# JoshuaLim007/VoxelEngine

Hardware: AMD Instinct MI355X
Metric: Mrays/s primary+1-bounce @1080p, 8k×512×8k brickmap; % HBM roofline (higher is better)
Workload: dtype f32

## Files before the change

### include/vxrt.h

```cpp
#ifndef VXRT_H
#define VXRT_H

#include <stddef.h>
#include <stdint.h>

#ifdef __cplusplus
extern "C" {
#endif

#define VXRT_ABI_VERSION 3
#define VXRT_EMPTY_SLOT 0xFFFFFFFFu
#define VXRT_MAX_STEPS 2048

typedef enum vxrt_status {
    VXRT_OK = 0,
    VXRT_ERR_INVALID = -1,
    VXRT_ERR_HIP = -2,
    VXRT_ERR_NO_WORLD = -3,
    VXRT_ERR_NOMEM = -4
} vxrt_status;

typedef struct vxrt_ctx vxrt_ctx;

int vxrt_abi_version(void);
int vxrt_create(int device, vxrt_ctx **out);
int vxrt_destroy(vxrt_ctx *ctx);
const char *vxrt_last_error(void);
int vxrt_synchronize(vxrt_ctx *ctx);
int vxrt_set_kernel_variant(vxrt_ctx *ctx, int variant);
int vxrt_debug_guard_pretend_no_slack(vxrt_ctx *ctx, int on);
int vxrt_has_experiments(void);
int vxrt_set_persistent_waves_per_cu(vxrt_ctx *ctx, int waves_per_cu);

typedef struct vxrt_world_desc {
    uint32_t struct_size;
    int32_t factor;
    int32_t cdims[3];
    uint64_t nslots;
    const uint32_t *coarse_bits;
    const uint32_t *brick_slot;
    const float *bounds;
    const uint32_t *pool;
} vxrt_world_desc;
int vxrt_upload_world(vxrt_ctx *ctx, const vxrt_world_desc *desc);

// ... 219 lines not shown
```

### voxelengine_amd/_native.py

```python
from __future__ import annotations

import ctypes as C
import os

from . import build as _build

EMPTY_SLOT = 0xFFFFFFFF
MAX_STEPS = 2048
GEN_HASH_HEIGHTFIELD, GEN_PERLIN_REF, GEN_INT_TERRAIN = 0, 1, 2
MODE_SHADED, MODE_DEBUG = 0, 1

EXPORTS = [
    "vxrt_abi_version", "vxrt_create", "vxrt_destroy", "vxrt_last_error", "vxrt_synchronize", "vxrt_set_kernel_variant", "vxrt_kernel_for_launch",
    "vxrt_has_experiments", "vxrt_set_persistent_waves_per_cu", "vxrt_debug_guard_pretend_no_slack",
    "vxrt_upload_world", "vxrt_build_world_procedural", "vxrt_world_info_get", "vxrt_download_world",
    "vxrt_save_world", "vxrt_load_world", "vxrt_world_file_info",
    "vxrt_set_environment", "vxrt_set_fov", "vxrt_set_ortho_window_size", "vxrt_get_directions",
    "vxrt_render_flags_default", "vxrt_render", "vxrt_render_views", "vxrt_compact_rows", "vxrt_frame_stats_get",
    "vxrt_deinterleave_strips", "vxrt_deinterleave_views", "vxrt_trace_batch", "vxrt_trace_batch_host",
    "vxrt_set_batch_max_steps", "vxrt_stream_open", "vxrt_stream_focus", "vxrt_stream_resident", "vxrt_stream_close",
    "vxrt_edit_voxels", "vxrt_edit_reserve",
    "vxrt_region_words", "vxrt_read_region", "vxrt_read_region_host", "vxrt_edit_stamps",
    "vxrt_move_boxes", "vxrt_overlap_boxes", "vxrt_move_boxes_host", "vxrt_overlap_boxes_host",
    "vxrt_islands_workspace_bytes", "vxrt_find_islands", "vxrt_find_islands_host",
    "vxrt_nav_workspace_bytes", "vxrt_nav_field", "vxrt_nav_paths", "vxrt_nav_field_host",
    "vxrt_distance_workspace_bytes", "vxrt_distance_field", "vxrt_distance_field_host",
]
EDIT_BOX, EDIT_SPHERE = 0, 1
EDIT_MAX_OPS = 1024
# ... 94 lines not shown
    path = os.environ.get("VXRT_LIB", _build.LIB_PATH)
    if path == _build.LIB_PATH:
        _build.build_lib(force=bool(os.environ.get("VXRT_REBUILD")))
    if not os.path.exists(path):
        raise RuntimeError(f"libvxrt.so not found at {path}; run __graft_entry__.build()")
    L = C.CDLL(path)
    f3 = C.POINTER(C.c_float)
    L.vxrt_abi_version.restype = C.c_int
    L.vxrt_last_error.restype = C.c_char_p
    L.vxrt_create.argtypes = [C.c_int, C.POINTER(C.c_void_p)]
    L.vxrt_destroy.argtypes = [C.c_void_p]
    L.vxrt_synchronize.argtypes = [C.c_void_p]
    L.vxrt_set_kernel_variant.argtypes = [C.c_void_p, C.c_int]
    L.vxrt_has_experiments.restype = C.c_int
    L.vxrt_debug_guard_pretend_no_slack.argtypes = [C.c_void_p, C.c_int]
    L.vxrt_set_persistent_waves_per_cu.argtypes = [C.c_void_p, C.c_int]
    L.vxrt_kernel_for_launch.argtypes = [C.c_void_p, C.c_uint32, C.c_uint32, C.c_void_p, C.c_uint32]
    L.vxrt_kernel_for_launch.restype = C.c_int
    L.vxrt_upload_world.argtypes = [C.c_void_p, C.POINTER(WorldDesc)]
    L.vxrt_build_world_procedural.argtypes = [C.c_void_p, C.c_int, C.c_int, C.c_int, C.c_int, C.c_int]
    L.vxrt_world_info_get.argtypes = [C.c_void_p, C.POINTER(WorldInfo)]
    L.vxrt_download_world.argtypes = [C.c_void_p, C.c_void_p, C.c_void_p, C.c_void_p, C.c_void_p]
    L.vxrt_save_world.argtypes = [C.c_void_p, C.c_char_p]
    L.vxrt_load_world.argtypes = [C.c_void_p, C.c_char_p]
    L.vxrt_world_file_info.argtypes = [C.c_char_p, C.POINTER(WorldInfo)]
    L.vxrt_set_environment.argtypes = [C.c_void_p, f3, f3, f3]
    L.vxrt_set_fov.argtypes = [C.c_void_p, C.c_float]
    L.vxrt_set_ortho_window_size.argtypes = [C.c_void_p, C.c_float, C.c_float]
    L.vxrt_get_directions.argtypes = [f3, f3, f3, f3]
    L.vxrt_get_directions.restype = None
# ... 66 lines not shown
```

### voxelengine_amd/csrc/vxrt_api.hip

```cpp
#include "../../include/vxrt.h"
#include "vxrt_dist.hpp"
#include "vxrt_edit.hpp"
#include "vxrt_kernels.hpp"
#include "vxrt_islands.hpp"
#include "vxrt_nav.hpp"
#include "vxrt_region.hpp"
#include "vxrt_stream.hpp"

#include <algorithm>
#include <atomic>
#include <cmath>
#include <cstdio>
#include <cstdlib>
#include <cstring>
#include <initializer_list>
#include <map>
#include <new>
#include <set>
#include <string>
#include <utility>
#include <vector>

namespace vxrt {
hipError_t launch_render(const RenderArgs& A, bool stats, int variant, hipStream_t stream);
int resolve_render_variant(const RenderArgs& A, int variant);
hipError_t launch_trace_batch(const BatchArgs& B, bool stats, int variant, hipStream_t stream);
void launch_deinterleave(const void* shards, unsigned long long shard_stride_bytes, void* fb, uint32_t width,
                         uint32_t height, uint32_t strip_rows, uint32_t strip_count, hipStream_t stream, uint32_t n_views = 1,
                         unsigned long long view_stride_bytes = 0, unsigned long long fb_stride_bytes = 0);
int build_world_on_device(struct ::vxrt_ctx* ctx, int generator, int X, int Y, int Z, int factor);
hipError_t layout_bits(const uint32_t* src, uint32_t* dst, const int cd[3], bool to_hbm);
hipError_t layout_meta(const uint2* src, uint2* dst, const int cd[3], bool to_hbm);
hipError_t layout_bricks(const uint32_t* src, uint32_t* dst, uint64_t nbricks, int f, bool to_hbm);
hipError_t chunk_tables(uint2* meta, uint32_t* coarse, const uint2* d_chunk_meta, int tx, int ty, int tz, int cx, int cz);
hipError_t edit_bricks(const uint32_t* cells, uint32_t n, const EditOpDev* ops, uint32_t nops, const uint2* meta,
                       const uint32_t* pool, uint32_t* scratch, uint32_t* ext, uint2* info, int f, int cx, int cz);
hipError_t edit_commit(const uint32_t* cells, const uint32_t* new_slot, uint32_t n, const uint32_t* zero, uint32_t nzero,
                       const uint32_t* scratch, const uint32_t* ext, uint32_t* pool, uint2* meta, uint32_t* coarse, int f);
hipError_t gather_bricks(const uint32_t* pool, const uint32_t* idx, uint32_t n, uint32_t* dst, int f);
hipError_t stamp_bricks(const uint32_t* cells, uint32_t n, const StampDev* stamps, uint32_t nst, const uint2* meta,
                        const uint32_t* pool, uint32_t* scratch, uint32_t* ext, uint2* info, int f, int cx, int cz);
hipError_t move_boxes(const CollideWorld& W, const float* bodies, uint64_t n, const int order[3], float* lohi, uint32_t* flags,
                      hipStream_t stream);
hipError_t overlap_boxes(const CollideWorld& W, const float* bodies, uint64_t n, uint32_t* counts, uint32_t* flags,
                         hipStream_t stream);
hipError_t find_islands(const CollideWorld& W, const int32_t o[3], const int32_t d[3], uint32_t anchors, void* work,
                        uint32_t* floating, uint32_t* labels, vxrt_island* table, uint32_t max_islands,
                        vxrt_island_summary* summary, hipStream_t stream);
hipError_t nav_field(const CollideWorld& W, const int32_t o[3], const int32_t d[3], const vxrt_nav_agent& ag, const int32_t* goals,
// ... 15 lines not shown
#define VX_HIP(call)                                                                                   \
    do {                                                                                               \
        hipError_t e_ = (call);                                                                        \
        if (e_ != hipSuccess)                                                                          \
            return fail(VXRT_ERR_HIP, std::string(#call) + ": " + hipGetErrorString(e_));              \
    } while (0)

struct vxrt_ctx {
    int device = 0;
    bool has_world = false;
    vxrt::WorldView view{};
    uint32_t* d_coarse = nullptr;
    void* coarse_alloc = nullptr;
    void* pool_alloc = nullptr;
    uint2* d_meta = nullptr;
    uint32_t* d_pool = nullptr;
    uint64_t ncells = 0, nslots = 0, pool_capacity_slots = 0;
    uint64_t coarse_alloc_bytes = 0, pool_alloc_bytes = 0;
    bool guard_no_slack = false;
    float light_dir[3] = {0, 0, 0};
    float light_color[3] = {0, 0, 0};
    float ambient[3] = {0, 0, 0};
    float fov = 90.0f;
    float ortho[2] = {10.0f, 10.0f};
    uint32_t frame_counter = 0;
    int kernel_variant = 4;
    unsigned persistent_waves = 4096;
    unsigned cus = 256;
    unsigned long long* d_stats = nullptr;
    unsigned int* d_queues = nullptr;
// ... 27 lines not shown
};
constexpr unsigned kViewSlots = 16;
constexpr unsigned kTileCounterRing = 64;
static_assert(kTileCounterRing == sizeof(vxrt_ctx::counter_busy) / sizeof(hipEvent_t), "ring size");
static_assert(kViewSlots == sizeof(vxrt_ctx::views_busy) / sizeof(hipEvent_t), "ring size");

namespace vxrt {

void stream_drop(vxrt_ctx* c);

static void free_world(vxrt_ctx* c)
{
    stream_drop(c);
    if (c->coarse_alloc) (void)hipFree(c->coarse_alloc);
    if (c->d_meta) (void)hipFree(c->d_meta);
    if (c->pool_alloc) (void)hipFree(c->pool_alloc);
    c->coarse_alloc = c->pool_alloc = nullptr;
    c->d_coarse = nullptr;
    c->d_meta = nullptr;
    c->d_pool = nullptr;
    c->has_world = false;
    c->ncells = c->nslots = c->pool_capacity_slots = 0;
    c->free_slots.clear();
    c->edited = false;
}

int check_shape(int factor, const int cd[3])
{
    if (!(factor == 8 || factor == 16 || factor == 32))
        return fail(VXRT_ERR_INVALID, "factor must be 8, 16 or 32");
    for (int a = 0; a < 3; ++a)
        if (cd[a] <= 0 || cd[a] % 8 != 0 || cd[a] > 65535)
            return fail(VXRT_ERR_INVALID, "coarse dimensions must be positive multiples of 8 (the tables' tiled order)");
    const uint64_t slice = (uint64_t)cd[0] * (uint64_t)cd[2];
    if ((uint64_t)cd[1] * (uint64_t)cd[2] >= (1ull << 24) || slice * (uint64_t)cd[1] + 2ull * slice + 64ull >= (1ull << 32))
        return fail(VXRT_ERR_INVALID, "coarse grid too large for 32-bit cell indices (cy * cz must stay below 2^24, cx * cz * (cy + 2) below 2^32)");
    return VXRT_OK;
}

void fill_view(vxrt_ctx* c, int factor, const int cd[3])
{
    WorldView& v = c->view;
    v.coarse_bits = c->d_coarse;
    v.cell_meta = c->d_meta;
    v.pool = c->d_pool;
    v.cx = cd[0];
    v.cy = cd[1];
    v.cz = cd[2];
    v.c_row = cd[0];
    v.c_slice = cd[0] * cd[2];
    v.f = factor;
    v.f_row = factor;
    v.f_slice = factor * factor;
    v.brick_words = (uint32_t)(factor * factor * factor / 32);
    v.ff = (float)factor;
    v.inv_f = 1.0f / (float)factor;
    v.wmax_x = (float)((double)cd[0] - 1e-6);
    v.wmax_y = (float)((double)cd[1] - 1e-6);
    v.wmax_z = (float)((double)cd[2] - 1e-6);
// ... 11 lines not shown
static hipError_t alloc_pool(uint64_t bw, uint64_t slots, void** alloc, uint64_t* alloc_bytes, uint32_t** pool)
{
    const uint64_t pool_bytes = (slots ? slots : 1) * bw * sizeof(uint32_t);
    const uint64_t pool_slack = (bw * sizeof(uint32_t) + 255) / 256 * 256;
    hipError_t e = hipMalloc(alloc, pool_bytes + 2 * pool_slack);
    if (e != hipSuccess)
        return e;
    *alloc_bytes = pool_bytes + 2 * pool_slack;
    *pool = reinterpret_cast<uint32_t*>(static_cast<unsigned char*>(*alloc) + pool_slack);
    return hipSuccess;
}

int alloc_world(vxrt_ctx* c, int factor, const int cd[3], uint64_t pool_slots)
{
    free_world(c);
    c->ncells = (uint64_t)cd[0] * cd[1] * cd[2];
    uint64_t bw = (uint64_t)factor * factor * factor / 32;
    const uint64_t coarse_bytes = ((c->ncells + 31) / 32) * sizeof(uint32_t);
    const uint64_t coarse_slack = (((uint64_t)cd[0] * cd[2] / 8 + 64) + 255) / 256 * 256;
    VX_HIP(hipMalloc(&c->coarse_alloc, coarse_bytes + 2 * coarse_slack));
    c->coarse_alloc_bytes = coarse_bytes + 2 * coarse_slack;
    c->d_coarse = reinterpret_cast<uint32_t*>(static_cast<unsigned char*>(c->coarse_alloc) + coarse_slack);
    VX_HIP(hipMalloc((void**)&c->d_meta, c->ncells * sizeof(uint2)));
    VX_HIP(alloc_pool(bw, pool_slots, &c->pool_alloc, &c->pool_alloc_bytes, &c->d_pool));
    c->pool_capacity_slots = pool_slots;
    return VXRT_OK;
}

int adopt_world(vxrt_ctx* c, int factor, const int cd[3], uint64_t nslots, uint32_t** d_coarse, uint2** d_meta,
                uint32_t** d_pool)
{
    int rc = alloc_world(c, factor, cd, nslots);
    if (rc)
        return rc;
    c->nslots = nslots;
    fill_view(c, factor, cd);
    c->has_world = true;
    *d_coarse = c->d_coarse;
// ... 171 lines not shown
#endif
}

int vxrt_debug_guard_pretend_no_slack(vxrt_ctx* c, int on)
{
    if (!c)
        return fail(VXRT_ERR_INVALID, "NULL context");
    c->guard_no_slack = on != 0;
    if (c->has_world) {
        const int cd[3] = {c->view.cx, c->view.cy, c->view.cz};
        vxrt::fill_view(c, c->view.f, cd);
    }
    return VXRT_OK;
}

int vxrt_set_kernel_variant(vxrt_ctx* c, int variant)
{
    if (!c || !(variant == 1 || variant == 4 || variant == 7))
        return fail(VXRT_ERR_INVALID, "variant must be 4 (default), 7 (the persistent kernels on the wave-level tracer: what the default runs) or 1 (straightforward per-lane loops, the cross-check)");
    c->kernel_variant = variant;
    return VXRT_OK;
}

int vxrt_synchronize(vxrt_ctx* c)
{
    if (!c)
        return fail(VXRT_ERR_INVALID, "ctx is NULL");
    VX_HIP(hipSetDevice(c->device));
    VX_HIP(hipDeviceSynchronize());
    return VXRT_OK;
// ... 76 lines not shown
    return vxrt::build_world_on_device(c, generator, X, Y, Z, factor);
}

int vxrt_world_info_get(vxrt_ctx* c, vxrt_world_info* out)
{
    if (!c || !out)
        return fail(VXRT_ERR_INVALID, "NULL argument");
    if (!c->has_world)
        return fail(VXRT_ERR_NO_WORLD, "no world resident");
    out->factor = c->view.f;
    out->cdims[0] = c->view.cx;
    out->cdims[1] = c->view.cy;
    out->cdims[2] = c->view.cz;
    out->ncells = c->ncells;
    out->nslots = c->nslots;
    out->hbm_bytes = ((c->ncells + 31) / 32) * 4 + c->ncells * sizeof(uint2) + c->nslots * c->view.brick_words * 4ull;
    return VXRT_OK;
}

int vxrt_download_world(vxrt_ctx* c, uint32_t* coarse_bits, uint32_t* brick_slot, float* bounds, uint32_t* pool)
{
    if (!c || !coarse_bits || !brick_slot || !bounds)
        return fail(VXRT_ERR_INVALID, "NULL argument");
    if (!c->has_world)
        return fail(VXRT_ERR_NO_WORLD, "no world resident");
    VX_HIP(hipSetDevice(c->device));
    VX_HIP(hipDeviceSynchronize());
    const int cd[3] = {c->view.cx, c->view.cy, c->view.cz};
    const uint64_t coarse_bytes = ((c->ncells + 31) / 32) * sizeof(uint32_t);
    const uint64_t bw = c->view.brick_words;
    const uint64_t piece = std::max<uint64_t>(1, (64ull << 20) / (bw * 4));
// ... 136 lines not shown
    const unsigned n = nviews ? nviews : 1u;
    for (unsigned v = 0; v < n; ++v) {
        if (!views[v].d_fb)
            return fail(VXRT_ERR_INVALID, "a view has no framebuffer");
        for (int a = 0; a < 3; ++a)
            if (!std::isfinite(views[v].origin[a]) || !std::isfinite(views[v].fwd[a]) || !std::isfinite(views[v].up[a]) ||
                !std::isfinite(views[v].right[a]))
                return fail(VXRT_ERR_INVALID, "camera origin / forward / up / right must be finite numbers");
    }
    if (fl->d_accum && nviews != 0)
        return fail(VXRT_ERR_INVALID, "temporal accumulation (d_accum) is per view: use vxrt_render");
    if (fl->d_accum && (reinterpret_cast<uintptr_t>(fl->d_accum) & 15u))
        return fail(VXRT_ERR_INVALID, "d_accum must be 16-byte aligned");
    VX_HIP(hipSetDevice(c->device));
    hipStream_t stream = (hipStream_t)fl->stream;

    vxrt::RenderArgs A;
    memset(&A, 0, sizeof(A));
    A.W = c->view;
    A.width = width;
    A.height = height;
    {
        float aspect = (float)width / (float)height;
        float fov = (float)((double)c->fov * 3.1415 / 180.0);
        A.kx = tanf(fov / 2.0f) * aspect;
        A.ky = tanf(fov / 2.0f);
        A.ratio = (float)width / (float)height;
        A.ortho_x = c->ortho[0];
        A.ortho_y = c->ortho[1];
    }
// ... 206 lines not shown
                              (hipStream_t)stream, n_views, view_stride_bytes, fb_stride_bytes);
    VX_HIP(hipGetLastError());
    return VXRT_OK;
}

int vxrt_trace_batch(vxrt_ctx* c, const float* d_origins, const float* d_dirs, uint64_t n, float* d_pos,
                     float* d_normal, int32_t* d_steps, uint8_t* d_hit, int64_t* d_voxel, vxrt_frame_stats* stats,
                     void* stream_)
{
    if (!c || (n && (!d_origins || !d_dirs || !d_pos || !d_normal || !d_steps)))
        return fail(VXRT_ERR_INVALID, "NULL argument");
    if (!c->has_world)
        return fail(VXRT_ERR_NO_WORLD, "no world resident");
    VX_HIP(hipSetDevice(c->device));
    hipStream_t stream = (hipStream_t)stream_;
    vxrt::BatchArgs B;
    memset(&B, 0, sizeof(B));
    B.W = c->view;
    B.origins = d_origins;
    B.dirs = d_dirs;
    B.n = n;
    B.pos = d_pos;
    B.normal = d_normal;
    B.steps = d_steps;
    B.hit = d_hit;
    B.voxel = (long long*)d_voxel;
    B.stats = c->d_stats;
    const unsigned tslot = c->launch_seq.fetch_add(1u) % kTileCounterRing;
    bool capturing = false;
    VX_HIP(vxrt::ring_acquire(c->counter_busy[tslot], stream, capturing));
// ... 455 lines not shown
    vxrt::fill_view(c, h.factor, cd);
    c->has_world = true;
    c->stream = S;
    return VXRT_OK;
}

int vxrt_stream_focus(vxrt_ctx* c, const float focus[3], float radius, vxrt_stream_stats* out)
{
    if (!c || !focus || !vxrt::StreamPolicy::focus_valid(focus, radius))
        return fail(VXRT_ERR_INVALID, "NULL argument, non-finite focus, or negative or NaN radius");
    StreamState* S = c->stream;
    if (!S)
        return fail(VXRT_ERR_NO_WORLD, "no streamed world (vxrt_stream_open)");
    VX_HIP(hipSetDevice(c->device));
    VX_HIP(hipDeviceSynchronize());
    StreamDeviceIO io(c, S);
    vxrt::StreamPolicy::Result r;
    const int rc = S->P.focus(focus, radius, S->brick_bytes, io, r);
    const hipError_t e = hipDeviceSynchronize();
    if (rc)
        return rc;
    if (e != hipSuccess)
        return fail(VXRT_ERR_HIP, std::string("hipDeviceSynchronize: ") + hipGetErrorString(e));
    if (out) {
        out->chunks_total = S->P.nchunks;
        out->chunks_occupied = S->P.chunks_occupied;
        out->chunks_resident = S->P.chunks_resident;
        out->bricks_resident = S->P.bricks_resident;
        out->chunks_loaded = r.loaded;
        out->chunks_evicted = r.evicted;
// ... 44 lines not shown
        return fail(VXRT_ERR_NOMEM, std::string("brick pool growth to ") + std::to_string(capacity) + " bricks: " + hipGetErrorString(e));
    }
    if (c->nslots)
        e = hipMemcpy(pool, c->d_pool, c->nslots * bw * 4, hipMemcpyDeviceToDevice);
    if (e == hipSuccess)
        e = hipDeviceSynchronize();
    if (e != hipSuccess) {
        (void)hipFree(alloc);
        return fail(VXRT_ERR_HIP, std::string("brick pool growth: ") + hipGetErrorString(e));
    }
    (void)hipFree(c->pool_alloc);
    c->pool_alloc = alloc;
    c->pool_alloc_bytes = alloc_bytes;
    c->d_pool = pool;
    c->pool_capacity_slots = capacity;
    const int cd[3] = {c->view.cx, c->view.cy, c->view.cz};
    fill_view(c, c->view.f, cd);
    return VXRT_OK;
}

template <class Op>
static void edit_cells(const std::vector<Op>& ops, int f, int cx, int cz, uint64_t ncells, std::vector<uint32_t>& cells)
{
    uint64_t total = 0;
    for (const Op& op : ops) {
        uint64_t v = 1;
        for (int a = 0; a < 3; ++a)
            v *= (uint64_t)(op.hi[a] / f - op.lo[a] / f + 1);
        total += v;
    }
// ... 76 lines not shown
        flags[i] = (uint8_t)info[i].y;
    }
    EditPlan P;
    edit_plan_slots(old_slot.data(), flags.data(), n, c->free_slots, c->nslots, P);
    if (P.changed == 0)
        return finish();
    int rc = VXRT_OK;
    if (P.nslots >= (1ull << 32) - 2)
        rc = fail(VXRT_ERR_NOMEM, "brick slots exhausted (32-bit slot numbers)");
    else if (P.nslots > c->pool_capacity_slots)
        rc = grow_pool(c, edit_grown_capacity(c->pool_capacity_slots, P.nslots));
    if (rc) {
        edit_plan_undo(P, c->free_slots);
        return rc;
    }
    uint32_t* d_new = static_cast<uint32_t*>(c->edit_plan.p);
    uint32_t* d_zero = d_new + n;
    std::vector<uint32_t> plan(P.new_slot);
    plan.insert(plan.end(), P.zero.begin(), P.zero.end());
    e = hipMemcpy(d_new, plan.data(), plan.size() * 4, hipMemcpyHostToDevice);
    if (e == hipSuccess)
        e = edit_commit(d_cells, d_new, n, d_zero, (uint32_t)P.zero.size(), d_img, d_ext, c->d_pool, c->d_meta, c->d_coarse, f);
    if (e == hipSuccess)
        e = hipDeviceSynchronize();
    if (e != hipSuccess) {
        edit_plan_undo(P, c->free_slots);
        return fail(VXRT_ERR_HIP, std::string("edit commit: ") + hipGetErrorString(e));
    }
    c->nslots = P.nslots;
    c->edited = true;
// ... 506 lines not shown
```

### voxelengine_amd/csrc/vxrt_device.hpp

```cpp
#pragma once

#include <hip/hip_runtime.h>
#include <stdint.h>

namespace vxrt {

constexpr int kMaxSteps = 2048;
constexpr uint32_t kEmptySlot = 0xFFFFFFFFu;
constexpr float kInf = __builtin_huge_valf();
constexpr float kFltEps = 1.1920928955078125e-7f;

struct f3 {
    float x, y, z;
};
__device__ __forceinline__ f3 mk3(float x, float y, float z) { return f3{x, y, z}; }
__device__ __forceinline__ f3 operator+(f3 a, f3 b) { return f3{a.x + b.x, a.y + b.y, a.z + b.z}; }
__device__ __forceinline__ f3 operator-(f3 a, f3 b) { return f3{a.x - b.x, a.y - b.y, a.z - b.z}; }
__device__ __forceinline__ f3 operator*(f3 a, float s) { return f3{a.x * s, a.y * s, a.z * s}; }
__device__ __forceinline__ float dot3(f3 a, f3 b) { return a.x * b.x + a.y * b.y + a.z * b.z; }
__device__ __forceinline__ float lo(float a, float b) { return a < b ? a : b; }
__device__ __forceinline__ float hi(float a, float b) { return a > b ? a : b; }
__device__ __forceinline__ f3 unit3(f3 v) { return v * (1.0f / sqrtf(dot3(v, v))); }

#ifndef VXRT_HOST_CHECK
// ... 20 lines not shown
__device__ __forceinline__ float div_rn(float a, float b, float y)
{
    const float q = a * y;
    return fmaf(fmaf(-b, q, a), y, q);
}
__device__ __forceinline__ bool ordinary(float x)
{
    return ((__float_as_uint(x) & 0x7FFFFFFFu) - 0x0D800000u) < (0x72000000u - 0x0D800000u);
}
__device__ __forceinline__ f3 unit3_ordinary(f3 v, float dd) { return v * rcp_rn(sqrt_rn(dd)); }
__device__ __forceinline__ f3 reflect3(f3 i, f3 n) { return i - (n * 2.0f) * dot3(n, i); }

struct WorldView {
    const uint32_t* __restrict__ coarse_bits;
    const uint2* __restrict__ cell_meta;
    const uint32_t* __restrict__ pool;
    int cx, cy, cz;
    int c_row, c_slice;
    int f;
    int f_row, f_slice;
    uint32_t brick_words;
    float ff;
    float inv_f;
    float wmax_x, wmax_y, wmax_z;
    int X, Y;
    int c_wide;
    const uint32_t *coarse_end, *coarse_lo, *coarse_hi;
    const uint32_t *pool_end, *pool_lo, *pool_hi;
};

#ifndef VXRT_FIELD_CAP_XZ
#define VXRT_FIELD_CAP_XZ 1020u
#define VXRT_FIELD_CAP_Y 508u
#endif
constexpr uint32_t kFieldCapXZ = VXRT_FIELD_CAP_XZ, kFieldCapY = VXRT_FIELD_CAP_Y;

__host__ __device__ inline bool grid_is_wide(int cx, int cy, int cz)
{
    return cx > (int)kFieldCapXZ || cz > (int)kFieldCapXZ || cy > (int)kFieldCapY || cx + cy + cz + 4 >= kMaxSteps;
}

#ifndef VXRT_QUEUE_SHARDS
#define VXRT_QUEUE_SHARDS 8
#endif
// ... 407 lines not shown
```

### voxelengine_amd/csrc/vxrt_wave2.hpp

```cpp
#pragma once

#include "vxrt_device.hpp"
#ifdef VXRT_HOST_DEBUG
#include <cstdio>
#include <cstdlib>
#endif

namespace vxrt {

enum : uint32_t { ST_WALK = 0u, ST_BOX = 1u, ST_END = 2u, ST_ENDHIT = 3u, ST_DONE = 4u, ST_IDLE = 5u };
__device__ __forceinline__ bool waits_for_end(uint32_t st) { return (st | 1u) == 3u; }
#ifndef VXRT_PROBE_GD
#define VXRT_PROBE_GD 0
#endif
#ifdef VXRT_HOST_CHECK
inline unsigned long long& host_unsuspected_exits() { static unsigned long long n = 0; return n; }
#endif

__device__ __forceinline__ f3 normal_decode(uint32_t c)
{
    float v = (c & 4u) ? -1.0f : 1.0f;
    uint32_t a = c & 3u;
    return mk3(a == 1u ? v : 0.0f, a == 2u ? v : 0.0f, a == 3u ? v : 0.0f);
}

__device__ __forceinline__ bool vote_run(int parked, int others, int num) { return parked * num >= max(others, 1); }
#ifndef VXRT_VOTE_END
#define VXRT_VOTE_END 2
// ... 128 lines not shown
        const uint32_t c23 = t_in == ny ? c2 : c3;
        code = t_in == nx ? c1 : c23;
        return !(t_out < vmax(t_in, 0.0f));
    }

    __device__ __forceinline__ void cells_of(const WorldView& W, bool fine, uint32_t r, int& x, int& y, int& z) const
    {
        const int dmx = fine ? W.f : W.cx, dmy = fine ? W.f : W.cy, dmz = fine ? W.f : W.cz;
        int fx = (int)rem_fx(r), fy = (int)rem_fy(r), fz = (int)rem_fz(r);
        if (WIDE) {
            const uint32_t oxz = cold[CF_OFF_XZ * 64], oy = cold[CF_OFF_Y * 64];
            fx += fine ? 0 : (int)(oxz & 0xFFFFu);
            fy += fine ? 0 : (int)oy;
            fz += fine ? 0 : (int)(oxz >> 16);
        }
        x = d.x > 0 ? dmx - 1 - fx : fx;
        y = d.y > 0 ? dmy - 1 - fy : fy;
        z = d.z > 0 ? dmz - 1 - fz : fz;
    }

    static __device__ __forceinline__ float fast_div(float x, float dv, float iv)
    {
        const float q = x * iv;
        return fmaf(fmaf(-q, dv, x), iv, q);
    }

    template <bool FINE>
    __device__ __forceinline__ void start_walk(const WorldView& W, const f3 s)
    {
        ws = s;
        const int dmx = FINE ? W.f : W.cx, dmy = FINE ? W.f : W.cy, dmz = FINE ? W.f : W.cz;
        const uint32_t row = (uint32_t)(FINE ? W.f_row : W.c_row), slice = (uint32_t)(FINE ? W.f_slice : W.c_slice);
        const uint32_t nx = 0u - (dn & 1u), ny = 0u - ((dn >> 1) & 1u), nz = 0u - (dn >> 2);
// ... 94 lines not shown
        cold[CF_START_Z * 64] = __float_as_uint(s0.z);
        cold[CF_LAST_CI * 64] = 0xFFFFFFFFu;
        cold[CF_TOTAL * 64] = 0u;
        special = !(fabsf(d.x) >= kMinFastDir && fabsf(d.y) >= kMinFastDir && fabsf(d.z) >= kMinFastDir) ||
                  __float_as_uint(s0.x) == 0x80000000u || __float_as_uint(s0.y) == 0x80000000u || __float_as_uint(s0.z) == 0x80000000u;
        dn = (d.x > 0 ? 0u : 1u) | (d.y > 0 ? 0u : 2u) | (d.z > 0 ? 0u : 4u);
        start_walk<false>(W, s0);
    }
    __device__ __forceinline__ void after_begin_ray(bool launched) { fine_m &= ~__ballot(launched); }

    __device__ __forceinline__ f3 cross_of(const WorldView& W, bool fine, uint32_t before, uint32_t dec, float t) const
    {
        int bx, by, bz;
        cells_of(W, fine, before, bx, by, bz);
        const bool on_x = dec == kRemDecX, on_y = dec == kRemDecY, on_z = dec == kRemDecZ;
        float face_x = (float)(bx + (d.x > 0 ? 1 : 0)), face_y = (float)(by + (d.y > 0 ? 1 : 0)), face_z = (float)(bz + (d.z > 0 ? 1 : 0));
        float lin_x = ws.x + (t * d.x), lin_y = ws.y + (t * d.y), lin_z = ws.z + (t * d.z);
        pin(face_x), pin(face_y), pin(face_z), pin(lin_x), pin(lin_y), pin(lin_z);
        return mk3(on_x ? face_x : lin_x, on_y ? face_y : lin_y, on_z ? face_z : lin_z);
    }

    __device__ __forceinline__ void walk_on(const WorldView& W, bool is_fine, bool lin_inside)
    {
        const bool single = t_hi == -kInf;
        if (__ballot(single) == 0ull)
            return;
        int x, y, z;
        cells_of(W, is_fine, rem, x, y, z);
        const int dmx = is_fine ? W.f : W.cx, dmy = is_fine ? W.f : W.cy, dmz = is_fine ? W.f : W.cz;
        const int row = is_fine ? W.f_row : W.c_row, slice = is_fine ? W.f_slice : W.c_slice;
        const uint32_t exact = cell_index(min(x, dmx - 1), min(y, dmy - 1), min(z, dmz - 1), row, dmz) + (uint32_t)slice;
// ... 18 lines not shown
            uint32_t offx = 0u, offy = 0u, offz = 0u;
            if (WIDE) {
                const uint32_t oxz = cold[CF_OFF_XZ * 64], oy = cold[CF_OFF_Y * 64];
                offx = oxz & 0xFFFFu;
                offy = oy;
                offz = oxz >> 16;
                const uint32_t off_k = dec_last == kRemDecX ? offx : (dec_last == kRemDecY ? offy : offz);
                virt = !is_fine && guard && stepped && off_k != 0u;
                exiting = exiting && !virt;
                exhausted = virt && !hit && rem0 - rem_sum(rp) + 1u >= (uint32_t)kMaxSteps;
            }
            const float F = W.ff;
            const f3 lin = mk3(ws.x + (tl * d.x), ws.y + (tl * d.y), ws.z + (tl * d.z));
            int bx, by, bz;
            cells_of(W, is_fine, rp, bx, by, bz);
            const f3 cr = mk3(dec_last == kRemDecX ? (float)(bx + (d.x > 0 ? 1 : 0)) : lin.x,
                              dec_last == kRemDecY ? (float)(by + (d.y > 0 ? 1 : 0)) : lin.y,
                              dec_last == kRemDecZ ? (float)(bz + (d.z > 0 ? 1 : 0)) : lin.z);
            float cr_lo = vmin3(cr.x, cr.y, cr.z), cr_hi = vmax3(cr.x, cr.y, cr.z);
            float lin_lo = vmin3(lin.x, lin.y, lin.z), lin_hi = vmax3(lin.x, lin.y, lin.z);
            f3 pc_prev = cross_of(W, is_fine, rpp, dec_prev, tp);
            pin(cr_lo), pin(cr_hi), pin(lin_lo), pin(lin_hi);
            const bool region_fail = is_fine & stepped & ((cr_lo < 0.0f) | (cr_hi > F));
            const bool resume = !hit && !exiting && !region_fail && !exhausted;
            if (resume) {
                if (WIDE) {
                    const uint32_t so_far = rem0 - rem_sum(rp) + 1u;
                    const uint32_t cap = ((uint32_t)kMaxSteps - so_far - 1u) / 3u;
                    const uint32_t tx = rem_fx(rp) + offx - (dec_last == kRemDecX ? 1u : 0u), ty = rem_fy(rp) + offy - (dec_last == kRemDecY ? 1u : 0u),
                                   tz = rem_fz(rp) + offz - (dec_last == kRemDecZ ? 1u : 0u);
                    const uint32_t px = min(tx, min(cap, kFieldCapXZ)), py = min(ty, min(cap, kFieldCapY)), pz = min(tz, min(cap, kFieldCapXZ));
                    const uint32_t armed = px | (py << 11) | (pz << 21);
                    if (virt) {
// ... 86 lines not shown
                }
            }
        }
        fine_m &= ~__ballot(go_coarse);
    }

    template <bool STATS = false>
    __device__ __forceinline__ void phase_box(const WorldView& W)
    {
        bool go_fine = false;
        if (st == ST_BOX) {
            int x, y, z;
            cells_of(W, false, rp, x, y, z);
            const int qx = min(x, W.cx - 1), qy = min(y, W.cy - 1), qz = min(z, W.cz - 1);
            const uint32_t ci = cell_index(qx, qy, qz, W.c_row, W.cz);
            const uint2 meta = W.cell_meta[ci];
            const uint32_t e = meta.y;
            const float fqx = (float)qx, fqy = (float)qy, fqz = (float)qz;
            f3 bmin = mk3(((float)(e & 31u) + 0) * W.inv_f + fqx, ((float)((e >> 5) & 31u) + 0) * W.inv_f + fqy,
                          ((float)((e >> 10) & 31u) + 0) * W.inv_f + fqz);
            f3 bmax = mk3(((float)((e >> 15) & 31u) + 1) * W.inv_f + fqx, ((float)((e >> 20) & 31u) + 1) * W.inv_f + fqy,
                          ((float)((e >> 25) & 31u) + 1) * W.inv_f + fqz);
            f3 bp;
            uint32_t bc;
            bool box_hit = slab_fast(ws, bmin, bmax, bp, bc) && bmin.x <= bmax.x;
            if (__ballot(special) != 0ull) {
                if (special)
                    box_hit = slab(ws, bmin, bmax, bp, bc) && bmin.x <= bmax.x;
            }
            if (box_hit) {
                const uint32_t steps = rem0 - rem_sum(rp);
                cold[CF_TOTAL * 64] += steps;
                if (STATS)
                    cnt.coarse_probes += steps + 1u;
                point.x = steps != 0u ? bp.x : ws.x;
                point.y = steps != 0u ? bp.y : ws.y;
                point.z = steps != 0u ? bp.z : ws.z;
                const bool enter = ci != cold[CF_LAST_CI * 64];
                if (enter) {
                    const uint32_t dec = rp - rem;
                    const int axis = dec == kRemDecX ? 0 : (dec == kRemDecY ? 1 : 2);
                    const int packed = axis | ((x - qx) << 2) | ((y - qy) << 3) | ((z - qz) << 4);
                    if (STATS)
                        cnt.brick_entries += 1u;
                    cold[CF_LAST_CI * 64] = ci;
                    cold[CF_CHX * 64] = (uint32_t)qx;
                    cold[CF_CHY * 64] = (uint32_t)qy;
                    cold[CF_CHZ * 64] = (uint32_t)qz;
                    cold[CF_BOX_CODES * 64] = bc | ((uint32_t)packed << 3);
                    const f3 hp = mk3(point.x * W.ff, point.y * W.ff, point.z * W.ff);
                    const f3 ns = mk3(hp.x - fqx * W.ff, hp.y - fqy * W.ff, hp.z - fqz * W.ff);
                    bits = W.pool + (size_t)meta.x * W.brick_words - (W.f_slice >> 5);
                    start_walk<true>(W, ns);
                    go_fine = true;
                } else {
                    st = ST_DONE;
                }
            } else {
                const bool left = (rem & kRemGuards) != 0u;
                if (!left)
                    walk_on(W, false, true);
                st = left ? (uint32_t)ST_END : (uint32_t)ST_WALK;
            }
        }
        fine_m |= __ballot(go_fine);
    }

// ... 217 lines not shown
```

### voxelengine_amd/csrc/vxrt_worldgen.hip

```cpp
#include "../../include/vxrt.h"
#include "vxrt_kernels.hpp"

#include <string>
#include <vector>

struct vxrt_ctx;

namespace vxrt {

int check_shape(int factor, const int cd[3]);
int alloc_world(vxrt_ctx* c, int factor, const int cd[3], uint64_t pool_slots);
void fill_view(vxrt_ctx* c, int factor, const int cd[3]);


__device__ __forceinline__ uint32_t g_hash32(uint32_t s)
{
    s = (s + 0x7ed55d16u) + (s << 12);
    s = (s ^ 0xc761c23cu) ^ (s >> 19);
    s = (s + 0x165667b1u) + (s << 5);
    s = (s + 0xd3a2646cu) ^ (s << 9);
    s = (s + 0xfd7046c5u) + (s << 3);
    s = (s ^ 0xb55a4f09u) ^ (s >> 16);
    return s;
}
// ... 171 lines not shown
        return;
    const uint32_t s = slot[cell];
    if (threadIdx.x == 0) {
        int bx, by, bz;
        ref_tiled_cell(cell, cx / 8, cy / 8, bx, by, bz);
        meta[hbm_index(bx, by, bz, cx, cz)] = make_uint2(s, ext[cell]);
    }
    if (s == kEmptySlot)
        return;
    const uint4* src = scratch + (size_t)cell * vecs_per_brick;
    uint4* dst = pool + (size_t)s * vecs_per_brick;
    for (uint32_t i = threadIdx.x; i < vecs_per_brick; i += blockDim.x)
        dst[i] = src[i];
}

__global__ void k_coarse_bits(const uint8_t* __restrict__ any, uint32_t* __restrict__ coarse, int cx, int cy, int cz)
{
    const uint64_t w = (uint64_t)blockIdx.x * blockDim.x + threadIdx.x;
    const uint64_t ncells = (uint64_t)cx * cy * cz, nwords = (ncells + 31) / 32;
    if (w >= nwords)
        return;
    uint32_t bits = 0;
    for (uint32_t k = 0; k < 32u; ++k) {
        const uint64_t i = w * 32u + k;
        if (i >= ncells)
            break;
        int x, y, z;
        hbm_cell(i, cx, cz, x, y, z);
        if (any[ref_tiled_index(x, y, z, cx / 8, cy / 8)])
            bits |= 1u << k;
// ... 107 lines not shown
    else
        hipLaunchKernelGGL(k_layout_meta<false>, g, b, 0, 0, src, dst, cd[0], cd[1], cd[2]);
    return hipGetLastError();
}
hipError_t layout_bricks(const uint32_t* src, uint32_t* dst, uint64_t nbricks, int f, bool to_hbm)
{
    const uint32_t words = (uint32_t)(f * f * f) / 32u;
    for (uint64_t done = 0; done < nbricks;) {
        const uint64_t n = nbricks - done < (1ull << 30) ? nbricks - done : (1ull << 30);
        if (to_hbm)
            hipLaunchKernelGGL(k_layout_bricks<true>, dim3((unsigned)n), dim3(256), 0, 0, src + done * words, dst + done * words, f);
        else
            hipLaunchKernelGGL(k_layout_bricks<false>, dim3((unsigned)n), dim3(256), 0, 0, src + done * words, dst + done * words, f);
        done += n;
    }
    return hipGetLastError();
}
hipError_t chunk_tables(uint2* meta, uint32_t* coarse, const uint2* d_chunk_meta, int tx, int ty, int tz, int cx, int cz)
{
    hipLaunchKernelGGL(k_chunk_tables, dim3(1), dim3(512), 0, 0, meta, coarse, d_chunk_meta, tx, ty, tz, cx, cz);
    return hipGetLastError();
}

}

namespace vxrt {

int adopt_world(vxrt_ctx* c, int factor, const int cd[3], uint64_t nslots, uint32_t** d_coarse, uint2** d_meta,
                uint32_t** d_pool);
int set_error(int code, const char* msg);
// ... 80 lines not shown
```

### voxelengine_amd/engine.py

```python
from __future__ import annotations

import ctypes as C
import os
from dataclasses import dataclass, field
from typing import NamedTuple

import numpy as np

from . import _native as N


def _f3(v):
    return (C.c_float * 3)(*[float(x) for x in v])


def GetDirections(euler):
    f, u, r = (C.c_float * 3)(), (C.c_float * 3)(), (C.c_float * 3)()
    N.load().vxrt_get_directions(_f3(euler), f, u, r)
    return (np.array(f[:], np.float32), np.array(u[:], np.float32), np.array(r[:], np.float32))


def tile_schedule(width: int, frame_rows, fwd, up, right, fov_deg: float = 90.0, height: int | None = None):
    frame_rows = np.asarray(list(frame_rows), np.int64)
    H = int(height if height is not None else (frame_rows.max() + 1 if frame_rows.size else 1))
# ... 414 lines not shown
        N.check(self._L.vxrt_trace_batch(self._h, _ptr(d_origins), _ptr(d_dirs), int(n), _ptr(d_pos), _ptr(d_normal),
                                         _ptr(d_steps), _ptr(d_hit), _ptr(d_voxel),
                                         C.byref(st) if want_stats else None, _stream(stream)))
        return st if want_stats else None

    def set_kernel_variant(self, variant: int) -> None:
        N.check(self._L.vxrt_set_kernel_variant(self._h, int(variant)))
        self.kernel_variant = int(variant)

    def set_persistent_waves_per_cu(self, waves_per_cu: int) -> None:
        N.check(self._L.vxrt_set_persistent_waves_per_cu(self._h, int(waves_per_cu)))

    def guard_pretend_no_slack(self, on: bool) -> None:
        N.check(self._L.vxrt_debug_guard_pretend_no_slack(self._h, int(bool(on))))

    def has_experiments(self) -> bool:
        return bool(self._L.vxrt_has_experiments())

    KERNEL_NAMES = {1: "k_render", 7: "k_render_persist2"}

    def kernel_for_launch(self, width: int, height: int, opts: "RenderOptions | None" = None, nviews: int = 0) -> int:
        fl = self._flags(opts, None)
        k = int(self._L.vxrt_kernel_for_launch(self._h, int(width), int(height), C.byref(fl), int(nviews)))
        if k < 0:
            raise N.VxrtError("vxrt_kernel_for_launch: bad arguments")
        return k

    def synchronize(self) -> None:
        N.check(self._L.vxrt_synchronize(self._h))

# ... 237 lines not shown
```

Baseline: 8531.

## Precompute per-cell float bounding boxes and use sign masks for face math

```diff
diff --git a/include/vxrt.h b/include/vxrt.h
--- a/include/vxrt.h
+++ b/include/vxrt.h
@@ -29,6 +29,8 @@
 int vxrt_synchronize(vxrt_ctx *ctx);
 int vxrt_set_kernel_variant(vxrt_ctx *ctx, int variant);
 int vxrt_debug_guard_pretend_no_slack(vxrt_ctx *ctx, int on);
+int vxrt_debug_cell_boxes(vxrt_ctx *ctx, uint32_t *cell_meta, uint32_t *cell_box);
+int vxrt_debug_edits_keep_box_generation(vxrt_ctx *ctx, int on);
 int vxrt_has_experiments(void);
 int vxrt_set_persistent_waves_per_cu(vxrt_ctx *ctx, int waves_per_cu);
 
diff --git a/voxelengine_amd/_native.py b/voxelengine_amd/_native.py
--- a/voxelengine_amd/_native.py
+++ b/voxelengine_amd/_native.py
@@ -13,6 +13,7 @@
 EXPORTS = [
     "vxrt_abi_version", "vxrt_create", "vxrt_destroy", "vxrt_last_error", "vxrt_synchronize", "vxrt_set_kernel_variant", "vxrt_kernel_for_launch",
     "vxrt_has_experiments", "vxrt_set_persistent_waves_per_cu", "vxrt_debug_guard_pretend_no_slack",
+    "vxrt_debug_cell_boxes", "vxrt_debug_edits_keep_box_generation",
     "vxrt_upload_world", "vxrt_build_world_procedural", "vxrt_world_info_get", "vxrt_download_world",
     "vxrt_save_world", "vxrt_load_world", "vxrt_world_file_info",
     "vxrt_set_environment", "vxrt_set_fov", "vxrt_set_ortho_window_size", "vxrt_get_directions",
@@ -137,6 +138,8 @@
     L.vxrt_set_kernel_variant.argtypes = [C.c_void_p, C.c_int]
     L.vxrt_has_experiments.restype = C.c_int
     L.vxrt_debug_guard_pretend_no_slack.argtypes = [C.c_void_p, C.c_int]
+    L.vxrt_debug_cell_boxes.argtypes = [C.c_void_p, C.c_void_p, C.c_void_p]
+    L.vxrt_debug_edits_keep_box_generation.argtypes = [C.c_void_p, C.c_int]
     L.vxrt_set_persistent_waves_per_cu.argtypes = [C.c_void_p, C.c_int]
     L.vxrt_kernel_for_launch.argtypes = [C.c_void_p, C.c_uint32, C.c_uint32, C.c_void_p, C.c_uint32]
     L.vxrt_kernel_for_launch.restype = C.c_int
diff --git a/voxelengine_amd/csrc/vxrt_api.hip b/voxelengine_amd/csrc/vxrt_api.hip
--- a/voxelengine_amd/csrc/vxrt_api.hip
+++ b/voxelengine_amd/csrc/vxrt_api.hip
@@ -33,6 +33,7 @@
 hipError_t layout_meta(const uint2* src, uint2* dst, const int cd[3], bool to_hbm);
 hipError_t layout_bricks(const uint32_t* src, uint32_t* dst, uint64_t nbricks, int f, bool to_hbm);
 hipError_t chunk_tables(uint2* meta, uint32_t* coarse, const uint2* d_chunk_meta, int tx, int ty, int tz, int cx, int cz);
+hipError_t cell_boxes(const uint2* meta, uint4* boxes, const int cd[3], float inv_f);
 hipError_t edit_bricks(const uint32_t* cells, uint32_t n, const EditOpDev* ops, uint32_t nops, const uint2* meta,
                        const uint32_t* pool, uint32_t* scratch, uint32_t* ext, uint2* info, int f, int cx, int cz);
 hipError_t edit_commit(const uint32_t* cells, const uint32_t* new_slot, uint32_t n, const uint32_t* zero, uint32_t nzero,
@@ -78,6 +79,9 @@
     void* coarse_alloc = nullptr;
     void* pool_alloc = nullptr;
     uint2* d_meta = nullptr;
+    uint4* d_boxes = nullptr;
+    uint64_t world_gen = 1, boxes_gen = 0;
+    bool debug_edits_keep_generation = false;
     uint32_t* d_pool = nullptr;
     uint64_t ncells = 0, nslots = 0, pool_capacity_slots = 0;
     uint64_t coarse_alloc_bytes = 0, pool_alloc_bytes = 0;
@@ -135,15 +139,35 @@
     stream_drop(c);
     if (c->coarse_alloc) (void)hipFree(c->coarse_alloc);
     if (c->d_meta) (void)hipFree(c->d_meta);
+    if (c->d_boxes) (void)hipFree(c->d_boxes);
     if (c->pool_alloc) (void)hipFree(c->pool_alloc);
     c->coarse_alloc = c->pool_alloc = nullptr;
     c->d_coarse = nullptr;
     c->d_meta = nullptr;
+    c->d_boxes = nullptr;
     c->d_pool = nullptr;
     c->has_world = false;
     c->ncells = c->nslots = c->pool_capacity_slots = 0;
     c->free_slots.clear();
     c->edited = false;
+}
+
+static void world_changed(vxrt_ctx* c) { c->world_gen += 1; }
+
+static int refresh_boxes(vxrt_ctx* c, hipStream_t stream)
+{
+    if (c->boxes_gen == c->world_gen)
+        return VXRT_OK;
+    hipStreamCaptureStatus cs = hipStreamCaptureStatusNone;
+    if (stream && hipStreamIsCapturing(stream, &cs) != hipSuccess)
+        (void)hipGetLastError();
+    if (cs != hipStreamCaptureStatusNone)
+        return fail(VXRT_ERR_INVALID, "the world has changed since the last launch: launch once outside the stream capture first");
+    const int cd[3] = {c->view.cx, c->view.cy, c->view.cz};
+    VX_HIP(cell_boxes(c->d_meta, c->d_boxes, cd, c->view.inv_f));
+    VX_HIP(hipDeviceSynchronize());
+    c->boxes_gen = c->world_gen;
+    return VXRT_OK;
 }
 
 int check_shape(int factor, const int cd[3])
@@ -164,6 +188,7 @@
     WorldView& v = c->view;
     v.coarse_bits = c->d_coarse;
     v.cell_meta = c->d_meta;
+    v.cell_box = c->d_boxes;
     v.pool = c->d_pool;
     v.cx = cd[0];
     v.cy = cd[1];
@@ -205,6 +230,7 @@
 int alloc_world(vxrt_ctx* c, int factor, const int cd[3], uint64_t pool_slots)
 {
     free_world(c);
+    world_changed(c);
     c->ncells = (uint64_t)cd[0] * cd[1] * cd[2];
     uint64_t bw = (uint64_t)factor * factor * factor / 32;
     const uint64_t coarse_bytes = ((c->ncells + 31) / 32) * sizeof(uint32_t);
@@ -213,6 +239,7 @@
     c->coarse_alloc_bytes = coarse_bytes + 2 * coarse_slack;
     c->d_coarse = reinterpret_cast<uint32_t*>(static_cast<unsigned char*>(c->coarse_alloc) + coarse_slack);
     VX_HIP(hipMalloc((void**)&c->d_meta, c->ncells * sizeof(uint2)));
+    VX_HIP(hipMalloc((void**)&c->d_boxes, c->ncells * 2 * sizeof(uint4)));
     VX_HIP(alloc_pool(bw, pool_slots, &c->pool_alloc, &c->pool_alloc_bytes, &c->d_pool));
     c->pool_capacity_slots = pool_slots;
     return VXRT_OK;
@@ -414,6 +441,29 @@
     return VXRT_OK;
 }
 
+int vxrt_debug_cell_boxes(vxrt_ctx* c, uint32_t* cell_meta, uint32_t* cell_box)
+{
+    if (!c || !cell_meta || !cell_box)
+        return fail(VXRT_ERR_INVALID, "NULL argument");
+    if (!c->has_world)
+        return fail(VXRT_ERR_NO_WORLD, "no world resident");
+    VX_HIP(hipSetDevice(c->device));
+    if (int rc = vxrt::refresh_boxes(c, nullptr))
+        return rc;
+    VX_HIP(hipDeviceSynchronize());
+    VX_HIP(hipMemcpy(cell_meta, c->d_meta, c->ncells * sizeof(uint2), hipMemcpyDeviceToHost));
+    VX_HIP(hipMemcpy(cell_box, c->d_boxes, c->ncells * 2 * sizeof(uint4), hipMemcpyDeviceToHost));
+    return VXRT_OK;
+}
+
+int vxrt_debug_edits_keep_box_generation(vxrt_ctx* c, int on)
+{
+    if (!c)
+        return fail(VXRT_ERR_INVALID, "NULL context");
+    c->debug_edits_keep_generation = on != 0;
+    return VXRT_OK;
+}
+
 int vxrt_set_kernel_variant(vxrt_ctx* c, int variant)
 {
     if (!c || !(variant == 1 || variant == 4 || variant == 7))
@@ -520,7 +570,7 @@
     out->cdims[2] = c->view.cz;
     out->ncells = c->ncells;
     out->nslots = c->nslots;
-    out->hbm_bytes = ((c->ncells + 31) / 32) * 4 + c->ncells * sizeof(uint2) + c->nslots * c->view.brick_words * 4ull;
+    out->hbm_bytes = ((c->ncells + 31) / 32) * 4 + c->ncells * (sizeof(uint2) + 2 * sizeof(uint4)) + c->nslots * c->view.brick_words * 4ull;
     return VXRT_OK;
 }
 
@@ -687,6 +737,9 @@
         return fail(VXRT_ERR_INVALID, "d_accum must be 16-byte aligned");
     VX_HIP(hipSetDevice(c->device));
     hipStream_t stream = (hipStream_t)fl->stream;
+
+    if (int rc = vxrt::refresh_boxes(c, stream))
+        return rc;
 
     vxrt::RenderArgs A;
     memset(&A, 0, sizeof(A));
@@ -923,6 +976,8 @@
         return fail(VXRT_ERR_NO_WORLD, "no world resident");
     VX_HIP(hipSetDevice(c->device));
     hipStream_t stream = (hipStream_t)stream_;
+    if (int rc = vxrt::refresh_boxes(c, stream))
+        return rc;
     vxrt::BatchArgs B;
     memset(&B, 0, sizeof(B));
     B.W = c->view;
@@ -1408,6 +1463,7 @@
         return fail(VXRT_ERR_NO_WORLD, "no streamed world (vxrt_stream_open)");
     VX_HIP(hipSetDevice(c->device));
     VX_HIP(hipDeviceSynchronize());
+    vxrt::world_changed(c);
     StreamDeviceIO io(c, S);
     vxrt::StreamPolicy::Result r;
     const int rc = S->P.focus(focus, radius, S->brick_bytes, io, r);
@@ -1482,6 +1538,7 @@
     c->pool_alloc_bytes = alloc_bytes;
     c->d_pool = pool;
     c->pool_capacity_slots = capacity;
+    world_changed(c);
     const int cd[3] = {c->view.cx, c->view.cy, c->view.cz};
     fill_view(c, c->view.f, cd);
     return VXRT_OK;
@@ -1588,6 +1645,8 @@
         edit_plan_undo(P, c->free_slots);
         return rc;
     }
+    if (!c->debug_edits_keep_generation)
+        world_changed(c);
     uint32_t* d_new = static_cast<uint32_t*>(c->edit_plan.p);
     uint32_t* d_zero = d_new + n;
     std::vector<uint32_t> plan(P.new_slot);
diff --git a/voxelengine_amd/csrc/vxrt_device.hpp b/voxelengine_amd/csrc/vxrt_device.hpp
--- a/voxelengine_amd/csrc/vxrt_device.hpp
+++ b/voxelengine_amd/csrc/vxrt_device.hpp
@@ -58,6 +58,7 @@
 struct WorldView {
     const uint32_t* __restrict__ coarse_bits;
     const uint2* __restrict__ cell_meta;
+    const uint4* __restrict__ cell_box;
     const uint32_t* __restrict__ pool;
     int cx, cy, cz;
     int c_row, c_slice;
@@ -72,6 +73,14 @@
     const uint32_t *coarse_end, *coarse_lo, *coarse_hi;
     const uint32_t *pool_end, *pool_lo, *pool_hi;
 };
+
+__host__ __device__ inline void cell_box_of(uint32_t e, int qx, int qy, int qz, float inv_f, f3& bmin, f3& bmax)
+{
+    const float fqx = (float)qx, fqy = (float)qy, fqz = (float)qz;
+    bmin = f3{((float)(e & 31u) + 0) * inv_f + fqx, ((float)((e >> 5) & 31u) + 0) * inv_f + fqy, ((float)((e >> 10) & 31u) + 0) * inv_f + fqz};
+    bmax = f3{((float)((e >> 15) & 31u) + 1) * inv_f + fqx, ((float)((e >> 20) & 31u) + 1) * inv_f + fqy,
+              ((float)((e >> 25) & 31u) + 1) * inv_f + fqz};
+}
 
 #ifndef VXRT_FIELD_CAP_XZ
 #define VXRT_FIELD_CAP_XZ 1020u
diff --git a/voxelengine_amd/csrc/vxrt_wave2.hpp b/voxelengine_amd/csrc/vxrt_wave2.hpp
--- a/voxelengine_amd/csrc/vxrt_wave2.hpp
+++ b/voxelengine_amd/csrc/vxrt_wave2.hpp
@@ -12,6 +12,12 @@
 __device__ __forceinline__ bool waits_for_end(uint32_t st) { return (st | 1u) == 3u; }
 #ifndef VXRT_PROBE_GD
 #define VXRT_PROBE_GD 0
+#endif
+#ifndef VXRT_BOX_TABLE
+#define VXRT_BOX_TABLE 1
+#endif
+#ifndef VXRT_SIGN_MASKS
+#define VXRT_SIGN_MASKS 1
 #endif
 #ifdef VXRT_HOST_CHECK
 inline unsigned long long& host_unsuspected_exits() { static unsigned long long n = 0; return n; }
@@ -170,9 +176,37 @@
             fy += fine ? 0 : (int)oy;
             fz += fine ? 0 : (int)(oxz >> 16);
         }
+#if VXRT_SIGN_MASKS
+        uint32_t mx, my, mz;
+        up_masks(mx, my, mz);
+        x = (int)(((uint32_t)fx ^ mx) + (mx & (uint32_t)dmx));
+        y = (int)(((uint32_t)fy ^ my) + (my & (uint32_t)dmy));
+        z = (int)(((uint32_t)fz ^ mz) + (mz & (uint32_t)dmz));
+#else
         x = d.x > 0 ? dmx - 1 - fx : fx;
         y = d.y > 0 ? dmy - 1 - fy : fy;
         z = d.z > 0 ? dmz - 1 - fz : fz;
+#endif
+    }
+    __device__ __forceinline__ void up_masks(uint32_t& mx, uint32_t& my, uint32_t& mz) const
+    {
+        mx = (dn & 1u) - 1u;
+        my = ((dn >> 1) & 1u) - 1u;
+        mz = (dn >> 2) - 1u;
+    }
+    __device__ __forceinline__ void faces_of(int bx, int by, int bz, float& face_x, float& face_y, float& face_z) const
+    {
+#if VXRT_SIGN_MASKS
+        uint32_t mx, my, mz;
+        up_masks(mx, my, mz);
+        face_x = (float)(bx - (int)mx);
+        face_y = (float)(by - (int)my);
+        face_z = (float)(bz - (int)mz);
+#else
+        face_x = (float)(bx + (d.x > 0 ? 1 : 0));
+        face_y = (float)(by + (d.y > 0 ? 1 : 0));
+        face_z = (float)(bz + (d.z > 0 ? 1 : 0));
+#endif
     }
 
     static __device__ __forceinline__ float fast_div(float x, float dv, float iv)
@@ -297,7 +331,8 @@
         int bx, by, bz;
         cells_of(W, fine, before, bx, by, bz);
         const bool on_x = dec == kRemDecX, on_y = dec == kRemDecY, on_z = dec == kRemDecZ;
-        float face_x = (float)(bx + (d.x > 0 ? 1 : 0)), face_y = (float)(by + (d.y > 0 ? 1 : 0)), face_z = (float)(bz + (d.z > 0 ? 1 : 0));
+        float face_x, face_y, face_z;
+        faces_of(bx, by, bz, face_x, face_y, face_z);
         float lin_x = ws.x + (t * d.x), lin_y = ws.y + (t * d.y), lin_z = ws.z + (t * d.z);
         pin(face_x), pin(face_y), pin(face_z), pin(lin_x), pin(lin_y), pin(lin_z);
         return mk3(on_x ? face_x : lin_x, on_y ? face_y : lin_y, on_z ? face_z : lin_z);
@@ -346,9 +381,9 @@
             const f3 lin = mk3(ws.x + (tl * d.x), ws.y + (tl * d.y), ws.z + (tl * d.z));
             int bx, by, bz;
             cells_of(W, is_fine, rp, bx, by, bz);
-            const f3 cr = mk3(dec_last == kRemDecX ? (float)(bx + (d.x > 0 ? 1 : 0)) : lin.x,
-                              dec_last == kRemDecY ? (float)(by + (d.y > 0 ? 1 : 0)) : lin.y,
-                              dec_last == kRemDecZ ? (float)(bz + (d.z > 0 ? 1 : 0)) : lin.z);
+            float face_x, face_y, face_z;
+            faces_of(bx, by, bz, face_x, face_y, face_z);
+            const f3 cr = mk3(dec_last == kRemDecX ? face_x : lin.x, dec_last == kRemDecY ? face_y : lin.y, dec_last == kRemDecZ ? face_z : lin.z);
             float cr_lo = vmin3(cr.x, cr.y, cr.z), cr_hi = vmax3(cr.x, cr.y, cr.z);
             float lin_lo = vmin3(lin.x, lin.y, lin.z), lin_hi = vmax3(lin.x, lin.y, lin.z);
             f3 pc_prev = cross_of(W, is_fine, rpp, dec_prev, tp);
@@ -465,13 +500,19 @@
             cells_of(W, false, rp, x, y, z);
             const int qx = min(x, W.cx - 1), qy = min(y, W.cy - 1), qz = min(z, W.cz - 1);
             const uint32_t ci = cell_index(qx, qy, qz, W.c_row, W.cz);
+            const float fqx = (float)qx, fqy = (float)qy, fqz = (float)qz;
+            f3 bmin, bmax;
+            uint32_t slot;
+#if VXRT_BOX_TABLE && !defined(VXRT_HOST_CHECK)
+            const uint4 b0 = W.cell_box[2 * (size_t)ci], b1 = W.cell_box[2 * (size_t)ci + 1];
+            bmin = mk3(__uint_as_float(b0.x), __uint_as_float(b0.y), __uint_as_float(b0.z));
+            bmax = mk3(__uint_as_float(b0.w), __uint_as_float(b1.x), __uint_as_float(b1.y));
+            slot = b1.z;
+#else
             const uint2 meta = W.cell_meta[ci];
-            const uint32_t e = meta.y;
-            const float fqx = (float)qx, fqy = (float)qy, fqz = (float)qz;
-            f3 bmin = mk3(((float)(e & 31u) + 0) * W.inv_f + fqx, ((float)((e >> 5) & 31u) + 0) * W.inv_f + fqy,
-                          ((float)((e >> 10) & 31u) + 0) * W.inv_f + fqz);
-            f3 bmax = mk3(((float)((e >> 15) & 31u) + 1) * W.inv_f + fqx, ((float)((e >> 20) & 31u) + 1) * W.inv_f + fqy,
-                          ((float)((e >> 25) & 31u) + 1) * W.inv_f + fqz);
+            cell_box_of(meta.y, qx, qy, qz, W.inv_f, bmin, bmax);
+            slot = meta.x;
+#endif
             f3 bp;
             uint32_t bc;
             bool box_hit = slab_fast(ws, bmin, bmax, bp, bc) && bmin.x <= bmax.x;
@@ -501,7 +542,7 @@
                     cold[CF_BOX_CODES * 64] = bc | ((uint32_t)packed << 3);
                     const f3 hp = mk3(point.x * W.ff, point.y * W.ff, point.z * W.ff);
                     const f3 ns = mk3(hp.x - fqx * W.ff, hp.y - fqy * W.ff, hp.z - fqz * W.ff);
-                    bits = W.pool + (size_t)meta.x * W.brick_words - (W.f_slice >> 5);
+                    bits = W.pool + (size_t)slot * W.brick_words - (W.f_slice >> 5);
                     start_walk<true>(W, ns);
                     go_fine = true;
                 } else {
diff --git a/voxelengine_amd/csrc/vxrt_worldgen.hip b/voxelengine_amd/csrc/vxrt_worldgen.hip
--- a/voxelengine_amd/csrc/vxrt_worldgen.hip
+++ b/voxelengine_amd/csrc/vxrt_worldgen.hip
@@ -209,6 +209,21 @@
         dst[i] = src[i];
 }
 
+__global__ __launch_bounds__(256) void k_cell_boxes(const uint2* __restrict__ meta, uint4* __restrict__ boxes, int cx, int cy, int cz,
+                                                    float inv_f)
+{
+    const uint64_t i = (uint64_t)blockIdx.x * blockDim.x + threadIdx.x;
+    if (i >= (uint64_t)cx * cy * cz)
+        return;
+    int x, y, z;
+    hbm_cell(i, cx, cz, x, y, z);
+    const uint2 m = meta[i];
+    f3 bmin, bmax;
+    cell_box_of(m.y, x, y, z, inv_f, bmin, bmax);
+    boxes[2u * i] = make_uint4(__float_as_uint(bmin.x), __float_as_uint(bmin.y), __float_as_uint(bmin.z), __float_as_uint(bmax.x));
+    boxes[2u * i + 1u] = make_uint4(__float_as_uint(bmax.y), __float_as_uint(bmax.z), m.x, 0u);
+}
+
 __global__ void k_coarse_bits(const uint8_t* __restrict__ any, uint32_t* __restrict__ coarse, int cx, int cy, int cz)
 {
     const uint64_t w = (uint64_t)blockIdx.x * blockDim.x + threadIdx.x;
@@ -346,6 +361,12 @@
             hipLaunchKernelGGL(k_layout_bricks<false>, dim3((unsigned)n), dim3(256), 0, 0, src + done * words, dst + done * words, f);
         done += n;
     }
+    return hipGetLastError();
+}
+hipError_t cell_boxes(const uint2* meta, uint4* boxes, const int cd[3], float inv_f)
+{
+    const uint64_t n = (uint64_t)cd[0] * cd[1] * cd[2];
+    hipLaunchKernelGGL(k_cell_boxes, dim3((unsigned)((n + 255) / 256)), dim3(256), 0, 0, meta, boxes, cd[0], cd[1], cd[2], inv_f);
     return hipGetLastError();
 }
 hipError_t chunk_tables(uint2* meta, uint32_t* coarse, const uint2* d_chunk_meta, int tx, int ty, int tz, int cx, int cz)
diff --git a/voxelengine_amd/engine.py b/voxelengine_amd/engine.py
--- a/voxelengine_amd/engine.py
+++ b/voxelengine_amd/engine.py
@@ -452,6 +452,16 @@
     def guard_pretend_no_slack(self, on: bool) -> None:
         N.check(self._L.vxrt_debug_guard_pretend_no_slack(self._h, int(bool(on))))
 
+    def debug_cell_boxes(self):
+        n = int(self.world_info().ncells)
+        meta = np.zeros((n, 2), np.uint32)
+        box = np.zeros((n, 8), np.uint32)
+        N.check(self._L.vxrt_debug_cell_boxes(self._h, meta.ctypes.data, box.ctypes.data))
+        return meta, box
+
+    def debug_edits_keep_box_generation(self, on: bool) -> None:
+        N.check(self._L.vxrt_debug_edits_keep_box_generation(self._h, int(bool(on))))
+
     def has_experiments(self) -> bool:
         return bool(self._L.vxrt_has_experiments())
 
```

Result: no change. 8610, median of 6 (+0.9%).
